# p768lwy3/torecsys

Measured on AMD Instinct MI355X. Metric: CTR samples/sec fwd+bwd (DeepFM, 39 fields x dim 64), higher is better.
Workload: dtype bf16; 1 GPU; BASELINE.json configs[1]: DeepFM 39 Criteo-shaped fields, MLP [400,400,400], 1000000 total rows, embed_dim 64, batch 65536, uniform indices, uniform field sizes; global_batch=65536, rows=1000000, parallelism=single, microbatches=1, optimizer=none, hipgraph=True, hipgraph_input_sets=1, hipgraph_steps_per_replay=4, fused_lookup_fm=True

## Files before the change

include/trs_abi.h:

```cpp
#ifndef TRS_ABI_H_
#define TRS_ABI_H_

#include <stddef.h>
#include <stdint.h>

#ifdef __cplusplus
extern "C" {
#endif

#define TRS_ABI_VERSION 3

enum { TRS_F32 = 0, TRS_BF16 = 1 };
enum { TRS_I64 = 0, TRS_I32 = 1 };
enum {
  TRS_OK = 0,
  TRS_EINVAL = -1,
  TRS_EDTYPE = -2,
  TRS_ESHAPE = -3,
  TRS_EALIGN = -4,
  TRS_ELAUNCH = -5,
  TRS_EWORKSPACE = -6
};

typedef void* trs_stream_t;
// ... 154 lines not shown
int trs_mlp_fused_fwd(const void* x, int64_t rows, int32_t num_layers, const int32_t* widths,
                      const void* const* weights, const void* const* biases, void* const* hidden, void* const* masks,
                      void* mask_in, void* y, int32_t dtype, int32_t family, int32_t x_stride, void* workspace,
                      size_t ws_bytes, trs_stream_t stream);
int trs_mlp_fused_bwd_data(const void* gy, int64_t rows, int32_t num_layers, const int32_t* widths,
                           const void* const* weights, const void* const* masks, void* const* gz, float* const* gbias,
                           void* gx, const void* mask_in, float* gbias_in, int32_t dtype, int32_t family,
                           void* workspace, size_t ws_bytes, trs_stream_t stream);

int trs_pad_cols(const void* src, int32_t c_in, void* dst, int32_t c_out, int64_t rows, int32_t dtype,
                 trs_stream_t stream);

size_t trs_rows_gemm_workspace_bytes(int32_t out_f, int32_t in_f);
int trs_rows_gemm_supported(int32_t out_f, int32_t in_f, int32_t x_stride);
int trs_rows_gemm(const void* x, int64_t rows, int32_t x_stride, const void* W, int32_t out_f, int32_t in_f,
                  int32_t dtype, void* y, void* workspace, size_t ws_bytes, trs_stream_t stream);

size_t trs_bucket_workspace_bytes(int64_t BN, int32_t world);
int trs_bucket_by_owner(const void* idx, int32_t idx_dtype, const int64_t* offsets, int64_t B, int32_t N,
                        int64_t rows_per_rank, int32_t world, int64_t* counts, int32_t* send_ids,
                        int32_t* send_pos, int32_t* inv_pos, void* workspace, size_t ws_bytes,
                        trs_stream_t stream);
int trs_embed_fm_sharded(const void* back, int64_t back_rows, const void* local, int64_t local_rows, int64_t n_valid,
                         int32_t E, int32_t dtype, const int32_t* inv_pos, const int32_t* send_ids, int32_t self_lo,
                         int32_t self_n, int64_t B, int32_t N, void* emb, void* fm, float* fm_sum, int32_t* err_flag,
                         trs_stream_t stream);
int trs_permute_grad(const void* g_block, const void* g_fm, const float* fm_sum, const void* x,
                     const int32_t* pos, int64_t K, int32_t N, int32_t E, int32_t dtype, void* out,
                     trs_stream_t stream);

int trs_rowdot_fwd(const void* h, const void* w, const void* bias, int64_t rows, int32_t C, int32_t dtype, void* out,
                   trs_stream_t stream);
size_t trs_rowdot_bwd_workspace_bytes(int64_t rows, int32_t C);
int trs_rowdot_bwd(const void* g, const void* h, const void* w, int64_t rows, int32_t C, int32_t dtype, void* gh,
                   float* gw, float* gb, void* workspace, size_t ws_bytes, trs_stream_t stream);

int trs_transpose_pad(const void* in, int64_t B, int32_t R, int32_t Cc, int32_t ld_in, void* out, int32_t ld_out,
                      int32_t dtype, trs_stream_t stream);

int trs_cat_head_fwd(const void* a, const void* d, const void* w, const void* bias, int64_t rows, int32_t N, int32_t Ea,
                     int32_t Eb, int32_t dtype, void* out, trs_stream_t stream);
size_t trs_cat_head_bwd_workspace_bytes(int64_t rows, int32_t N, int32_t Ea, int32_t Eb);
int trs_cat_head_bwd(const void* g, const void* a, const void* d, const void* w, int64_t rows, int32_t N, int32_t Ea,
                     int32_t Eb, int32_t dtype, void* ga, void* gd, float* gw, float* gb, void* workspace,
                     size_t ws_bytes, trs_stream_t stream);

int trs_wgrad_finish(const float* part, int32_t S, int32_t R, int32_t Cc, int32_t out_rows, int32_t out_cols,
                     int32_t dtype, void* gw, const float* gb_f32, void* gb, trs_stream_t stream);
int trs_wgrad_finish_t(const float* part, int32_t S, int32_t Cc, int32_t R, int32_t out_rows, int32_t out_cols,
                       int32_t dtype, void* gw, const float* gb_f32, void* gb, trs_stream_t stream);
int32_t trs_wgrad_rows_splits(int32_t M, int32_t N, int64_t rows);
int trs_wgrad_rows(const void* g, int32_t ldg, const void* x, int32_t ldx, int64_t rows, int32_t M, int32_t N,
                   int32_t dtype, int32_t S, float* part, trs_stream_t stream);
int trs_copy_padded_many(const int64_t* desc, int32_t n, int32_t elem_size, int64_t max_elems, trs_stream_t stream);

int32_t trs_cin_glue_blocks(int64_t B);
int trs_cin_glue_stats(const void* y, int64_t B, int32_t E, int32_t C, int32_t dtype, float* partial,
                       trs_stream_t stream);
int trs_cin_glue_fwd(const void* y, const float* scale, const float* shift, int64_t B, int32_t E, int32_t C, int32_t D,
                     int32_t Hs, int32_t dtype, void* hidden, void* pooled, trs_stream_t stream);
int trs_cin_glue_bwd_reduce(const void* y, const void* g_hidden, const void* g_pooled, const float* scale,
                            const float* shift, const float* mean, const float* invstd, int64_t B, int32_t E, int32_t C,
                            int32_t D, int32_t Hs, int32_t dtype, float* partial, trs_stream_t stream);
int trs_cin_glue_bwd_apply(const void* y, const void* g_hidden, const void* g_pooled, const float* scale,
                           const float* shift, const float* mean, const float* invstd, const float* c1, const float* c2,
                           int64_t B, int32_t E, int32_t C, int32_t D, int32_t Hs, int32_t dtype, void* gy,
                           trs_stream_t stream);
int trs_cin_glue_cf_supported(int32_t E, int32_t C);
int trs_cin_glue_fwd_cf(const void* y, const float* scale, const float* shift, int64_t B, int32_t E, int32_t C,
                        int32_t D, int32_t Hs, int32_t dtype, void* hidden, void* hidden_cf, void* pooled,
                        trs_stream_t stream);
int trs_cin_glue_bwd_apply_cf(const void* y, const void* g_hidden, const void* g_pooled, const float* scale,
                              const float* shift, const float* mean, const float* invstd, const float* c1,
                              const float* c2, int64_t B, int32_t E, int32_t C, int32_t D, int32_t Hs, int32_t dtype,
                              void* gy, void* gy_cf, float* colsum_partial, trs_stream_t stream);

int trs_opn_vec_fwd(const void* x, const void* kern, int32_t kern_is_num, int64_t B, int32_t N, int32_t E,
                    int32_t dtype, void* out, trs_stream_t stream);
size_t trs_opn_vec_bwd_workspace_bytes(int64_t B, int32_t N, int32_t E);
int trs_opn_vec_bwd(const void* g, const void* x, const void* kern, int32_t kern_is_num, int64_t B, int32_t N,
                    int32_t E, int32_t dtype, void* gx, float* gkern_vec, void* workspace, size_t ws_bytes,
                    trs_stream_t stream);

int trs_pair_mul_fwd(const void* a, const void* c, const void* bias, int32_t bias_per_pair, int64_t B, int32_t N,
                     int32_t E, int32_t dtype, void* out, trs_stream_t stream);
int trs_pair_mul_bwd(const void* g, const void* a, const void* c, int64_t B, int32_t N, int32_t E, int32_t dtype,
                     void* ga, void* gc, trs_stream_t stream);

int trs_rows_mul_bias_fwd(const void* a, const void* c, const void* bias, int32_t bias_per_pair, int64_t rows,
                          int32_t P, int32_t E, int32_t dtype, void* out, trs_stream_t stream);
int trs_rows_mul_bwd(const void* g, const void* a, const void* c, int64_t rows, int32_t E, int32_t dtype, void* ga,
                     void* gc, trs_stream_t stream);

int trs_pair_bilinear_fwd(const void* x, const void* W, int32_t w_per_pair, const void* bias, int32_t bias_per_pair,
                          int32_t mode, int64_t B, int32_t N, int32_t E, int32_t dtype, void* out,
                          trs_stream_t stream);
int trs_pair_bilinear_bwd_data(const void* g, const void* x, const void* W, int32_t w_per_pair, int32_t mode,
                               int64_t B, int32_t N, int32_t E, int32_t dtype, void* gx, void* gT,
                               trs_stream_t stream);

int trs_pair_bilinear_fwd_mfma(const void* x, const void* Wt, const void* bias, const int32_t* tasks, int32_t ntasks,
                               int32_t mode, int64_t B, int32_t N, int32_t E, int32_t dtype, void* out,
                               trs_stream_t stream);

int trs_pair_bilinear_bwd_data_mfma(const void* g, const void* x, const void* W, const void* Wt,
                                    const int32_t* tasks_i, int32_t nti, const int32_t* seg_i,
// ... 78 lines not shown
```

torecsys_amd/_abi.py:

```python
from __future__ import annotations

import ctypes
import os
import threading
from ctypes import c_char_p, c_int32, c_int64, c_size_t, c_void_p

import torch

_HERE = os.path.dirname(os.path.abspath(__file__))
LIB_PATH = os.environ.get("TRS_LIB_PATH") or os.path.join(_HERE, "libtrs_hip.so")

TRS_F32, TRS_BF16 = 0, 1
TRS_I64, TRS_I32 = 0, 1

_P, _I32, _I64, _SZ, _F32 = c_void_p, c_int32, c_int64, c_size_t, ctypes.c_float

_OPTIMIZER_TAIL = [_I32, _F32, _P, _F32, _F32, _F32, _P, _P, _P, _SZ, _P]

SIGNATURES = {
    "trs_version": (c_int32, []),
    "trs_last_error_string": (c_char_p, []),
    "trs_rowdot_fwd": (c_int32, [_P, _P, _P, _I64, _I32, _I32, _P, _P]),
    "trs_rowdot_bwd_workspace_bytes": (_SZ, [_I64, _I32]),
    "trs_rowdot_bwd": (c_int32, [_P, _P, _P, _I64, _I32, _I32, _P, _P, _P, _P, _SZ, _P]),
    "trs_transpose_pad": (c_int32, [_P, _I64, _I32, _I32, _I32, _P, _I32, _I32, _P]),
    "trs_cat_head_fwd": (c_int32, [_P, _P, _P, _P, _I64, _I32, _I32, _I32, _I32, _P, _P]),
    "trs_cat_head_bwd_workspace_bytes": (_SZ, [_I64, _I32, _I32, _I32]),
    "trs_cat_head_bwd": (c_int32, [_P, _P, _P, _P, _I64, _I32, _I32, _I32, _I32, _P, _P, _P, _P, _P, _SZ, _P]),
    "trs_wgrad_finish": (c_int32, [_P, _I32, _I32, _I32, _I32, _I32, _I32, _P, _P, _P, _P]),
    "trs_wgrad_finish_t": (c_int32, [_P, _I32, _I32, _I32, _I32, _I32, _I32, _P, _P, _P, _P]),
    "trs_wgrad_rows_splits": (c_int32, [_I32, _I32, _I64]),
    "trs_wgrad_rows": (c_int32, [_P, _I32, _P, _I32, _I64, _I32, _I32, _I32, _I32, _P, _P]),
    "trs_copy_padded_many": (c_int32, [_P, _I32, _I32, _I64, _P]),
    "trs_cin_glue_blocks": (c_int32, [_I64]),
    "trs_cin_glue_stats": (c_int32, [_P, _I64, _I32, _I32, _I32, _P, _P]),
    "trs_cin_glue_fwd": (c_int32, [_P, _P, _P, _I64, _I32, _I32, _I32, _I32, _I32, _P, _P, _P]),
    "trs_cin_glue_bwd_reduce": (c_int32, [_P, _P, _P, _P, _P, _P, _P, _I64, _I32, _I32, _I32, _I32, _I32, _P, _P]),
    "trs_cin_glue_bwd_apply": (c_int32, [_P, _P, _P, _P, _P, _P, _P, _P, _P, _I64, _I32, _I32, _I32, _I32, _I32, _P, _P]),
    "trs_cin_glue_cf_supported": (c_int32, [_I32, _I32]),
    "trs_cin_glue_fwd_cf": (c_int32, [_P, _P, _P, _I64, _I32, _I32, _I32, _I32, _I32, _P, _P, _P, _P]),
    "trs_cin_glue_bwd_apply_cf": (c_int32, [_P, _P, _P, _P, _P, _P, _P, _P, _P, _I64, _I32, _I32, _I32, _I32, _I32, _P, _P, _P,
                                            _P]),
    "trs_opn_vec_fwd": (c_int32, [_P, _P, _I32, _I64, _I32, _I32, _I32, _P, _P]),
    "trs_opn_vec_bwd_workspace_bytes": (_SZ, [_I64, _I32, _I32]),
    "trs_opn_vec_bwd": (c_int32, [_P, _P, _P, _I32, _I64, _I32, _I32, _I32, _P, _P, _P, _SZ, _P]),
    "trs_pair_mul_fwd": (c_int32, [_P, _P, _P, _I32, _I64, _I32, _I32, _I32, _P, _P]),
    "trs_rows_mul_bias_fwd": (c_int32, [_P, _P, _P, _I32, _I64, _I32, _I32, _I32, _P, _P]),
    "trs_rows_mul_bwd": (c_int32, [_P, _P, _P, _I64, _I32, _I32, _P, _P, _P]),
    "trs_pair_mul_bwd": (c_int32, [_P, _P, _P, _I64, _I32, _I32, _I32, _P, _P, _P]),
    "trs_pair_bilinear_fwd": (c_int32, [_P, _P, _I32, _P, _I32, _I32, _I64, _I32, _I32, _I32, _P, _P]),
    "trs_pair_bilinear_bwd_data": (c_int32, [_P, _P, _P, _I32, _I32, _I64, _I32, _I32, _I32, _P, _P, _P]),
    "trs_pair_bilinear_fwd_mfma": (c_int32, [_P, _P, _P, _P, _I32, _I32, _I64, _I32, _I32, _I32, _P, _P]),
    "trs_pair_bilinear_bwd_data_mfma": (c_int32, [_P, _P, _P, _P, _P, _I32, _P, _P, _I32, _P, _I32, _I64, _I32, _I32, _I32,
                                                  _P, _P, _P, _P]),
    "trs_pair_bilinear_bwd_w_mfma_workspace_bytes": (_SZ, [_I64, _I32, _I32]),
    "trs_pair_bilinear_bwd_w_mfma": (c_int32, [_P, _P, _I32, _I64, _I32, _I32, _I32, _P, _P, _SZ, _P]),
    "trs_pair_epilogue_fwd": (c_int32, [_P, _P, _P, _I32, _I32, _I64, _I32, _I32, _I32, _P, _P]),
    "trs_pair_epilogue_bwd": (c_int32, [_P, _P, _P, _I32, _I64, _I32, _I32, _I32, _P, _P]),
    "trs_afm_fwd_dropout": (c_int32, [_P, _P, _P, _P, _P, _P, _F32, _I64, _I32, _I32, _I32, _I32, _P, _P, _P, _P]),
    "trs_afm_bwd_dropout": (c_int32, [_P, _P, _P, _P, _P, _F32, _P, _P, _P, _I64, _I32, _I32, _I32, _I32, _P, _P, _P, _P,
                                      _P, _P, _SZ, _P]),
    "trs_afm_pair_tiles": (c_int32, [_I32, _P, _I32, _P]),
    "trs_pad_cols": (c_int32, [_P, _I32, _P, _I32, _I64, _I32, _P]),
    "trs_rows_gemm_workspace_bytes": (_SZ, [_I32, _I32]),
    "trs_rows_gemm_supported": (c_int32, [_I32, _I32, _I32]),
    "trs_rows_gemm": (c_int32, [_P, _I64, _I32, _P, _I32, _I32, _I32, _P, _P, _SZ, _P]),
    "trs_afm_bwd_workspace_bytes": (_SZ, [_I64, _I32, _I32, _I32]),
    "trs_pack_columns": (c_int32, [_P, _P, _I32, _I32, _I64, _P, _I32, _P]),
    "trs_mark_timestamp": (c_int32, [_P, _I32, _P]),
    "trs_wall_clock_khz": (_I64, []),
    "trs_gather_rows": (c_int32, [_P, _I64, _I32, _I32, _P, _I32, _P, _I64, _I32, _P, _P, _P]),
    "trs_gather_rows_tables": (c_int32, [_P, _P, _I32, _I32, _P, _I32, _I64, _I32, _P, _P, _P]),
    "trs_fa_gather_rows": (c_int32, [_P, _I64, _I32, _I32, _P, _I32, _P, _I64, _I32, _P, _P, _P]),
    "trs_csr_workspace_bytes": (_SZ, [_I64, _I64]),
    "trs_csr_build": (c_int32, [_P, _I32, _P, _I64, _I32, _I64, _P, _P, _P, _SZ, _P, _P]),
    "trs_csr_build_skip": (c_int32, [_P, _I32, _P, _I64, _I32, _I64, _I64, _P, _P, _P, _SZ, _P, _P]),
    "trs_scatter_workspace_bytes": (_SZ, [_I64, _I32, _I32, _I32]),
    "trs_scatter_rows": (c_int32, [_P, _I64, _P, _I32, _P, _P, _P, _P, _I64, _I64, _I32, _I32, _I32, _I64, _P, _P, _SZ, _P]),
    "trs_scatter_rows_first": (c_int32, [_P, _I64, _P, _I32, _P, _P, _P, _P, _I64, _I64, _I32, _I32, _I32, _I64, _P, _P, _P, _P,
                                         _SZ, _P]),
    "trs_scatter_rows_update": (c_int32, [_P, _I64, _P, _I32, _P, _P, _P, _P, _I64, _I64, _I32, _I32, _I32, _I64,
                                          *_OPTIMIZER_TAIL]),
    "trs_scatter_rows_update_mapped": (c_int32, [_P, _P, _P, _P, _P, _I64, _I64, _I64, _I32, _I32, *_OPTIMIZER_TAIL]),
    "trs_adam_step_size": (c_int32, [_P, _P, ctypes.c_double, ctypes.c_double, _P, _P]),
    "trs_compact_rows_slots": (_I64, [_I64]),
# ... 281 lines not shown
```

torecsys_amd/csrc/wgrad_rows.hip:

```cpp
#include <algorithm>

#include "trs_common.hpp"

namespace trs {

typedef __attribute__((ext_vector_type(4))) short wg_s16x4;
typedef __attribute__((ext_vector_type(8))) short wg_s16x8;
typedef __attribute__((ext_vector_type(8))) __bf16 wg_bf16x8;
typedef __attribute__((ext_vector_type(4))) float wg_f32x4;

constexpr int WG_KR = 64;
constexpr int WG_KS = 32;
constexpr int WG_PANEL = WG_KS * 32 + 32;
constexpr int WG_TC = 7;

struct WgradArgs {
  const uint16_t* g;
  const uint16_t* x;
  float* part;
  int64_t rows;
  int ldg, ldx;
  int M, N;
  int MB, NB;
  int slots_per_xcd;
};

__host__ __device__ __forceinline__ int split_start(int total, int parts, int k) { return (int)(((int64_t)total * k) / parts); }

__device__ __forceinline__ wg_bf16x8 tr_frag(const char* lo_p, const char* hi_p, int off) {
  typedef __attribute__((address_space(3))) wg_s16x4* lds_p;
  const wg_s16x4 lo = __builtin_amdgcn_ds_read_tr16_b64_v4i16((lds_p)(lo_p + off));
  const wg_s16x4 hi = __builtin_amdgcn_ds_read_tr16_b64_v4i16((lds_p)(hi_p + off));
  const wg_s16x8 v = {lo[0], lo[1], lo[2], lo[3], hi[0], hi[1], hi[2], hi[3]};
  return __builtin_bit_cast(wg_bf16x8, v);
}

__device__ __forceinline__ void wg_mfma(wg_f32x4& acc, const wg_bf16x8& A, const wg_bf16x8& B) {
  asm volatile("v_mfma_f32_16x16x32_bf16 %0, %1, %2, %0" : "+a"(acc) : "v"(A), "v"(B));
}

template <int WM, int WN, int MC, int NC, bool CHECK>
__global__ __launch_bounds__(64 * WM * WN, 1) void wgrad_rows_kernel(WgradArgs a) {
  constexpr int NWAVES = WM * WN;
  constexpr bool EXACT = NWAVES == 8;
  extern __shared__ __attribute__((aligned(16))) char wg_lds[];
  const int lane = threadIdx.x & 63, wave = __builtin_amdgcn_readfirstlane(threadIdx.x >> 6);
  const int q = lane >> 4, i = lane & 15;
  const bool odd = q & 1;

  const int TB = a.MB * a.NB;
  const int xcd = blockIdx.x & 7, j = blockIdx.x >> 3;
  const int slot = xcd * a.slots_per_xcd + j / TB;
  const int S = 8 * a.slots_per_xcd;
  const int tile = j % TB;
  const int mb = tile / a.NB, nb = tile % a.NB;
  const int Mt = (a.M + 15) >> 4, Nt = (a.N + 15) >> 4;
  const int bm0 = split_start(Mt, a.MB, mb), bm1 = split_start(Mt, a.MB, mb + 1);
  const int bn0 = split_start(Nt, a.NB, nb), bn1 = split_start(Nt, a.NB, nb + 1);
  const int PM = bm1 - bm0, PN = bn1 - bn0, P = PM + PN;
  const int wm = wave / WN, wn = (EXACT && wave >= 4) ? ((wave + 1) & 3) : wave % WN;
  const int am0 = split_start(PM, WM, wm), mc = split_start(PM, WM, wm + 1) - am0;
  const int an0 = split_start(PN, WN, wn), nc = split_start(PN, WN, wn + 1) - an0;
  const int64_t quads_total = (a.rows + 4 * WG_KS - 1) / (4 * WG_KS);
  const int64_t h0 = 4 * (quads_total * slot / S), h1 = 4 * (quads_total * (slot + 1) / S);
  const int64_t n_h = h1 - h0;

  constexpr int NLD = 32 / NWAVES;
  const int panel = (wave & 3) * 8 + ((lane & 15) >> 1);
  const int rlow = (wave >> 2) * 16 + (lane >> 4), half = lane & 1;
  const bool is_g = panel < PM;
  const int col = is_g ? 16 * (bm0 + panel) + 8 * half : 16 * (bn0 + panel - PM) + 8 * half;
  const bool col_ok = panel < P && col + 8 <= (is_g ? a.M : a.N);
  const int ld = is_g ? a.ldg : a.ldx;
  const uint16_t* src = (is_g ? a.g : a.x) + col;
  const int lds_off = panel * WG_PANEL + rlow * 32 + half * 16;
  const int slot_bytes = P * WG_PANEL;

// ... 219 lines not shown
      }                                                                                                             \
      landed();                                                                                                     \
      cur = nx;                                                                                                     \
    }
    if (n_h > 0) {
#pragma unroll
      for (int k = 0; k < WD_AHEAD; ++k) issue(k, k);
      landed();
      {
        const char* cb = wg_lds;
#pragma unroll
        for (int n = 0; n < NCx; ++n) Bf[n] = tr_frag(cb + b_lo, cb + b_hi, n * 32);
#pragma unroll
        for (int m = 0; m < PD; ++m) Ar[m] = tr_frag(cb + a_lo, cb + a_hi, m * 32);
      }
      for (int64_t k = 0; k < n_h; k += 4) {
        WD_STEP(0, k)
        WD_STEP(1, k + 1)
        WD_STEP(2, k + 2)
        WD_STEP(3, k + 3)
      }
    }
#undef WD_STEP
    asm volatile("s_waitcnt vmcnt(0)\n\ts_nop 15\n\ts_nop 15" ::: "memory");
    float* out = a.part + (int64_t)slot * a.M * a.N;
#pragma unroll
    for (int m = 0; m < MCx; ++m)
#pragma unroll
      for (int n = 0; n < NCx; ++n)
        if (m < mc && n < nc) {
          const int row = 16 * (bm0 + am0 + m) + 4 * q, c = 16 * (bn0 + an0 + n) + i;
#pragma unroll
          for (int e = 0; e < 4; ++e)
            if (row + e < a.M && c < a.N) out[(int64_t)(row + e) * a.N + c] = acc[m][n][e];
        }
  };
  if (mc == MC && nc == NC) run.template operator()<MC, NC>();
  else if (mc == MC) run.template operator()<MC, NC - 1>();
  else if (nc == NC) run.template operator()<MC - 1, NC>();
  else run.template operator()<MC - 1, NC - 1>();
}

constexpr int WD2_SLOT = 3 * WD_IMG;
constexpr int WD2_NSLOT = 4;
constexpr int WD2_AHEAD = 3;
constexpr int64_t WD2_MIN_ROWS = 1 << 20;

template <bool AG>
__device__ __forceinline__ void wd_mfma(wg_f32x4& acc, const wg_bf16x8& A, const wg_bf16x8& B) {
  if constexpr (AG) asm volatile("v_mfma_f32_16x16x32_bf16 %0, %1, %2, %0" : "+a"(acc) : "v"(A), "v"(B));
  else asm volatile("v_mfma_f32_16x16x32_bf16 %0, %1, %2, %0" : "+v"(acc) : "v"(A), "v"(B));
}

__global__ __launch_bounds__(256, 1) void wgrad_dma2_kernel(WgradArgs a) {
  extern __shared__ __attribute__((aligned(16))) char wg_lds[];
  const int lane = threadIdx.x & 63, wave = __builtin_amdgcn_readfirstlane(threadIdx.x >> 6);
  const int q = lane >> 4, i = lane & 15;
  const bool odd = q & 1;
  const int TB = a.MB;
  const int xcd = blockIdx.x & 7, j = blockIdx.x >> 3;
  const int slot = xcd * a.slots_per_xcd + j / TB;
  const int S = 8 * a.slots_per_xcd;
  const int mb = j % TB;
  const int Mt = (a.M + 15) >> 4, Nt = (a.N + 15) >> 4;
  const int bm0 = split_start(Mt, a.MB, mb), PM = split_start(Mt, a.MB, mb + 1) - bm0;
  const int xb = wave >> 1;
  const int bn0 = split_start(Nt, 2, xb), PN = split_start(Nt, 2, xb + 1) - bn0;
  const int an0 = split_start(PN, 2, wave & 1), nc = split_start(PN, 2, (wave & 1) + 1) - an0;
  const int xc0 = 16 * split_start(Nt, 2, 0), xc1 = 16 * split_start(Nt, 2, 1);
  const int64_t quads_total = a.rows / (4 * WG_KS);
  const int64_t h0 = 4 * (quads_total * slot / S), h1 = 4 * (quads_total * (slot + 1) / S);
  const int64_t n_h = h1 - h0;

  const char* gcol = reinterpret_cast<const char*>(a.g + 16 * bm0);
  const char* x0col = reinterpret_cast<const char*>(a.x + xc0);
  const char* x1col = reinterpret_cast<const char*>(a.x + xc1);
  unsigned voff[10];
#pragma unroll
  for (int t = 0; t < 10; ++t) {
    const int p = wave + 4 * t, img = p / 13, jj = p - 13 * img;
    const int o = jj * 1024 + 16 * lane, row = o / WD_S, cb = o - row * WD_S;
    voff[t] = (unsigned)(row * (img ? a.ldx : a.ldg) * 2 + cb);
  }
  const unsigned lds0 = (unsigned)(uintptr_t)(__attribute__((address_space(3))) const char*)wg_lds;
  auto issue = [&](int64_t k, unsigned ring_slot) __attribute__((always_inline)) {
    const int64_t h = h0 + (k < n_h ? k : n_h - 1);
    const char* gs = gcol + h * WG_KS * a.ldg * 2;
    const char* x0s = x0col + h * WG_KS * a.ldx * 2;
    const char* x1s = x1col + h * WG_KS * a.ldx * 2;
    const unsigned base = lds0 + ring_slot * WD2_SLOT;
#pragma unroll
    for (int t = 0; t < 10; ++t) {
      const int p = wave + 4 * t;
      if (p < 39) wd_dma(p < 13 ? gs : (p < 26 ? x0s : x1s), voff[t], base + p * 1024);
    }
  };
  auto landed = [&]() __attribute__((always_inline)) {
    if (wave < 3) asm volatile("s_waitcnt vmcnt(10) lgkmcnt(0)\n\ts_barrier" ::: "memory");
    else asm volatile("s_waitcnt vmcnt(9) lgkmcnt(0)\n\ts_barrier" ::: "memory");
  };

  auto run = [&]<int MCx, int NCx>() __attribute__((always_inline)) {
    wg_f32x4 acc[MCx][NCx];
#pragma unroll
    for (int m = 0; m < MCx; ++m)
#pragma unroll
      for (int n = 0; n < NCx; ++n) acc[m][n] = wg_f32x4{0.f, 0.f, 0.f, 0.f};
    const int frag_lane = (8 * q + (i >> 2)) * WD_S + (i & 3) * 8;
    const int a_lo = frag_lane + (odd ? 4 * WD_S : 0), a_hi = frag_lane + (odd ? 0 : 4 * WD_S);
    const int b_lo = WD_IMG * (1 + xb) + an0 * 32 + frag_lane + (odd ? 4 * WD_S : 0);
    const int b_hi = WD_IMG * (1 + xb) + an0 * 32 + frag_lane + (odd ? 0 : 4 * WD_S);
    constexpr int PD = 2;
    wg_bf16x8 Ar[4], Bf[NCx];
#define WD2_STEP(c4, KEXPR)                                                                                         \
    {                                                                                                               \
      const char* cb = wg_lds + (c4) * WD2_SLOT;                                                                    \
// ... 70 lines not shown
    if (p.MB * p.NB > 32) return WgradPlan{0, 0, 0, 0, 0, 0, 0};
    if (((Nt + p.NB - 1) / p.NB + 1) / 2 <= 5) p.nc = 5;
    const int pm_lo = Mt / p.MB, pm_hi = (Mt + p.MB - 1) / p.MB, pn_lo = Nt / p.NB, pn_hi = (Nt + p.NB - 1) / p.NB;
    if (pm_lo >= 12 && pm_hi <= 14 && pn_lo >= 12 && pn_hi <= 16) {
      p.wn = 4;
      p.mc = 7;
      p.nc = 4;
    } else if (pm_lo >= 12 && pm_hi <= 14 && pn_lo >= 8 && pn_hi <= 12) {
      p.wn = 4;
      p.mc = 7;
      p.nc = 3;
    }
  }
  auto blocks_ok = [](int T, int B, int cols) {
    for (int b = 0; b < B; ++b) {
      const int t0 = split_start(T, B, b), t1 = split_start(T, B, b + 1);
      if (t1 - t0 < 12 || t1 - t0 > 13 || 16 * t0 + 208 > cols) return false;
    }
    return true;
  };
  if (p.wm == 2 && p.wn == 4 && p.nc == 4 && rows % (4 * WG_KS) == 0 && blocks_ok(Mt, p.MB, M) &&
      blocks_ok(Nt, p.NB, N))
    p.dma = (p.NB == 2 && rows >= WD2_MIN_ROWS) ? 2 : 1;
  int slots = 32 / (p.dma == 2 ? p.MB : p.MB * p.NB);
  const int64_t stages = (rows + WG_KR - 1) / WG_KR;
  while (slots > 1 && stages / (8 * slots) < 4) slots >>= 1;
  p.slots_per_xcd = slots;
  return p;
}

template <int WM, int WN, int MC, int NC, bool CHECK>
int wgrad_launch_c(const WgradArgs& a, int grid, size_t lds, hipStream_t s) {
  static bool attr = false;
  if (!attr) {
    if (hipFuncSetAttribute((const void*)wgrad_rows_kernel<WM, WN, MC, NC, CHECK>, hipFuncAttributeMaxDynamicSharedMemorySize,
                            160 * 1024) != hipSuccess)
      return check_launch("wgrad_rows: LDS attribute");
    attr = true;
  }
  hipLaunchKernelGGL((wgrad_rows_kernel<WM, WN, MC, NC, CHECK>), dim3(grid), dim3(64 * WM * WN), lds, s, a);
  return check_launch("wgrad_rows");
}

}

using namespace trs;

template <int WM, int WN, int MC, int NC>
static int wgrad_launch(const WgradArgs& a, int grid, size_t lds, hipStream_t s) {
  return (a.rows % (4 * WG_KS)) ? wgrad_launch_c<WM, WN, MC, NC, true>(a, grid, lds, s)
                          : wgrad_launch_c<WM, WN, MC, NC, false>(a, grid, lds, s);
}

extern "C" int32_t trs_wgrad_rows_splits(int32_t M, int32_t N, int64_t rows) {
  const WgradPlan p = wgrad_plan(M, N, rows);
  return 8 * p.slots_per_xcd;
}

extern "C" int trs_wgrad_rows(const void* g, int32_t ldg, const void* x, int32_t ldx, int64_t rows, int32_t M, int32_t N,
                              int32_t dtype, int32_t S, float* part, trs_stream_t stream) {
  TRS_REQUIRE(dtype == TRS_BF16, TRS_EDTYPE, "wgrad_rows: bf16 operands only");
  WgradPlan p = wgrad_plan(M, N, rows);
  TRS_REQUIRE(p.slots_per_xcd > 0 && S == 8 * p.slots_per_xcd, TRS_ESHAPE,
              "wgrad_rows: (M=%d, N=%d, rows=%lld) takes %d row ranges, caller passed %d", M, N, (long long)rows,
              8 * p.slots_per_xcd, S);
  TRS_REQUIRE(ldg >= M && ldx >= N && (ldg & 7) == 0 && (ldx & 7) == 0 && aligned16(g) && aligned16(x), TRS_ESHAPE,
              "wgrad_rows: row strides must be multiples of 8 elements and cover M / N, operands 16-byte aligned");
  if (!g || !x || !part) return fail(TRS_EINVAL, "wgrad_rows: null pointer");
  hipStream_t s = (hipStream_t)stream;
  WgradArgs a{(const uint16_t*)g, (const uint16_t*)x, part, rows, ldg, ldx, M, N, p.MB, p.NB, p.slots_per_xcd};
  const int Mt = (M + 15) / 16, Nt = (N + 15) / 16;
  const int PM = (Mt + p.MB - 1) / p.MB, PN = (Nt + p.NB - 1) / p.NB;
  const size_t lds = (size_t)(4 * (PM + PN) + WG_TC) * WG_PANEL;
  const int grid = 8 * p.slots_per_xcd * p.MB * p.NB;
  TRS_REQUIRE(p.dma == 0 || (int64_t)WG_KS * std::max(ldg, ldx) * 2 < ((int64_t)1 << 31), TRS_ESHAPE, "wgrad_rows: row stride too large");
  if (p.dma == 2) {
    static bool attr2 = false;
    if (!attr2) {
      if (hipFuncSetAttribute((const void*)wgrad_dma2_kernel, hipFuncAttributeMaxDynamicSharedMemorySize, 160 * 1024) != hipSuccess)
        return check_launch("wgrad_rows(dma2): LDS attribute");
      attr2 = true;
    }
    hipLaunchKernelGGL(wgrad_dma2_kernel, dim3(8 * p.slots_per_xcd * p.MB), dim3(256), (size_t)WD2_NSLOT * WD2_SLOT, s, a);
    return check_launch("wgrad_rows(dma2)");
  }
  if (p.dma == 1) {
    static bool attr = false;
    if (!attr) {
      if (hipFuncSetAttribute((const void*)wgrad_dma_kernel<7, 4>, hipFuncAttributeMaxDynamicSharedMemorySize, 160 * 1024) != hipSuccess)
        return check_launch("wgrad_rows(dma): LDS attribute");
      attr = true;
    }
    hipLaunchKernelGGL((wgrad_dma_kernel<7, 4>), dim3(grid), dim3(512), (size_t)WD_NSLOT * WD_SLOT, s, a);
    return check_launch("wgrad_rows(dma)");
  }
  if (p.wm == 2 && p.wn == 4)
    return p.nc == 4 ? wgrad_launch<2, 4, 7, 4>(a, grid, lds, s) : wgrad_launch<2, 4, 7, 3>(a, grid, lds, s);
  if (p.wm == 2)
    return p.nc == 5 ? wgrad_launch<2, 2, WG_TC, 5>(a, grid, lds, s) : wgrad_launch<2, 2, WG_TC, WG_TC>(a, grid, lds, s);
  if (p.wm == 4) return p.nc == 4 ? wgrad_launch<4, 1, WG_TC, 4>(a, grid, lds, s) : wgrad_launch<4, 1, WG_TC, WG_TC>(a, grid, lds, s);
  if (p.mc == 1) return wgrad_launch<1, 4, 1, WG_TC>(a, grid, lds, s);
  if (p.mc == 4) return wgrad_launch<1, 4, 4, WG_TC>(a, grid, lds, s);
  return wgrad_launch<1, 4, WG_TC, WG_TC>(a, grid, lds, s);
}
```

torecsys_amd/layers.py:

```python
from __future__ import annotations

from abc import ABC, abstractmethod
from typing import Dict, List, Optional, Tuple

import math
import os

import torch
import torch.nn as nn

from . import functional as F_


def _strip(t: torch.Tensor) -> torch.Tensor:
    return t.rename(None) if t.has_names() else t


class BaseLayer(nn.Module, ABC):

    def __init__(self, **kwargs):
        super().__init__()

    @property
    @abstractmethod
# ... 583 lines not shown
    def forward(ctx, x, weight, bias, fuse_relu, w_pad, b_pad):
        W = weight if w_pad is None else w_pad
        Bv = bias if w_pad is None else b_pad
        x2 = x.reshape(-1, x.shape[-1])
        if fuse_relu and Bv is not None and x2.is_cuda:
            y = torch._addmm_activation(Bv, x2, W.t(), use_gelu=False).reshape(*x.shape[:-1], W.shape[0])
        else:
            y = torch.nn.functional.linear(x, W, Bv)
            if fuse_relu:
                y = torch.relu_(y)
        ctx.has_bias = bias is not None
        ctx.fuse_relu = bool(fuse_relu) and bias is not None and F_.relu_bwd_bias_supported(y.reshape(-1, y.shape[-1]))
        ctx.relu = bool(fuse_relu)
        ctx.wshape = tuple(weight.shape)
        ctx.wdtype = weight.dtype
        ctx.save_for_backward(x, W, y if fuse_relu else None)
        return y

    @staticmethod
    def backward(ctx, g):
        x, W, y = ctx.saved_tensors
        out_f, in_f = ctx.wshape
        gx = gw = gb = None
        if ctx.fuse_relu:
            gz, gbf = F_.relu_bwd_bias(g.reshape(-1, g.shape[-1]), y.reshape(-1, y.shape[-1]))
            g = gz.reshape(g.shape)
            gb = gbf[:out_f].to(ctx.wdtype)
        elif ctx.relu:
            g = g * (y > 0).to(g.dtype)
        g2 = g.reshape(-1, g.shape[-1])
        x2 = x.reshape(-1, x.shape[-1])
        if ctx.needs_input_grad[0]:
            gx = (g2 @ W).reshape(x.shape)
        if ctx.needs_input_grad[1]:
            rows, S = g2.shape[0], _split_count(g2.shape[0], _LinearSplitK.SPLIT_ROWS)
            if S >= 4 and rows % S == 0 and 32 <= g2.shape[1] <= 1024 and 32 <= x2.shape[1] <= 1024 \
                    and g2.is_contiguous() and x2.is_contiguous():
                part = torch.bmm(g2.view(S, rows // S, -1).transpose(1, 2), x2.view(S, rows // S, -1),
                                 out_dtype=torch.float32)
                gw = part.sum(0)[:out_f, :in_f].to(ctx.wdtype)
            else:
                gw = (g2.t() @ x2)[:out_f, :in_f]
                if not gw.is_contiguous():
                    gw = gw.contiguous()
        if ctx.has_bias and ctx.needs_input_grad[2] and gb is None:
            rows = g2.shape[0]
            if g2.shape[1] <= 8 and rows % 1024 == 0 and rows >= 8192 and g2.is_contiguous():
                gb = g2.view(rows // 1024, 1024, -1).float().sum(1).sum(0)[:out_f].to(g2.dtype)
            else:
                gb = g2.sum(0)[:out_f]
        return gx, gw, gb, None, None, None


def _dense_layer_grads(g2, gbf, xin, W, out_f, in_f, wdt, need_x, need_w, need_b):
    rows = xin.shape[0]
    gw_out = gb_out = None
    S = _split_count(rows, _LinearSplitK.SPLIT_ROWS)
    if need_w or (need_b and gbf is not None):
        if need_w and S >= 4 and rows % S == 0 and 32 <= g2.shape[1] <= 1024 and 32 <= xin.shape[1] <= 4096 \
                and xin.is_contiguous():
            gw = torch.empty(out_f, in_f, dtype=wdt, device=xin.device)
            St = _split_count(rows, _MLPStack.SPLIT_ROWS_WIDE)
            if xin.shape[1] >= 2 * g2.shape[1] and St >= 4:
                part = torch.bmm(xin.view(St, rows // St, -1).transpose(1, 2), g2.view(St, rows // St, -1),
                                 out_dtype=torch.float32)
                with_b = need_b and gbf is not None
                gb = torch.empty(out_f, dtype=wdt, device=xin.device) if with_b else None
                F_.call("trs_wgrad_finish_t", F_.ptr(part), St, part.shape[1], part.shape[2], out_f, in_f,
                        F_.value_dtype_code(gw), F_.ptr(gw), F_.ptr(gbf) if with_b else F_.ptr(None), F_.ptr(gb),
                        F_.stream_ptr())
            else:
                part = torch.bmm(g2.view(S, rows // S, -1).transpose(1, 2), xin.view(S, rows // S, -1),
                                 out_dtype=torch.float32)
                with_b = need_b and gbf is not None and out_f <= (in_f + 255) // 256 * 256
                gb = torch.empty(out_f, dtype=wdt, device=xin.device) if with_b else None
                F_.call("trs_wgrad_finish", F_.ptr(part), S, part.shape[1], part.shape[2], out_f, in_f,
                        F_.value_dtype_code(gw), F_.ptr(gw), F_.ptr(gbf) if with_b else F_.ptr(None), F_.ptr(gb),
                        F_.stream_ptr())
            gw_out = gw
            if with_b:
                gb_out = gb
        elif need_w:
            gw = (g2.t() @ xin)[:out_f, :in_f]
            gw_out = gw if gw.is_contiguous() else gw.contiguous()
    if need_b and gb_out is None:
        gb_out = gbf[:out_f].to(wdt) if gbf is not None else g2.sum(0)[:out_f]
    gx = None
    if need_x and F_.rows_gemm_supported(g2, W, out_f, xin.shape[1]) and W.shape[1] == xin.shape[1]:
        gx = F_.rows_gemm(g2, W, out_f, xin.shape[1])
    elif need_x:
        gx = g2 @ W
    return gx, gw_out, gb_out


class _HybridMLP(torch.autograd.Function):

    @staticmethod
    def forward(ctx, x, w_narrow, *tensors):
        cur = x.reshape(-1, x.shape[-1])
        w1, b1, w1u, b1u = tensors[:4]
        tail = tensors[4:]
        W1 = w1 if w1u is None else w1u
        B1 = b1 if w1u is None else b1u
        L = len(tail) // 4
        Ws = [(tail[4 * l] if tail[4 * l + 2] is None else tail[4 * l + 2]).contiguous() for l in range(L)]
        bs = [(tail[4 * l + 1] if tail[4 * l + 3] is None else tail[4 * l + 3]).contiguous() for l in range(L)]
        h1 = torch._addmm_activation(B1, cur, W1.t(), use_gelu=False)
        if w_narrow is not None:
            y, hidden, masks, mask_in, fam = F_.fused_mlp_forward_raw(h1, [w_narrow] + Ws[1:], bs, input_mask=True,
                                                                      family=F_.MLP_FAMILY_MIXED, x_stride=h1.shape[1])
        else:
            y, hidden, masks, mask_in, fam = F_.fused_mlp_forward_raw(h1, Ws, bs, input_mask=True)
# ... 425 lines not shown
```

Before: 58.94 million samples/s.

## Route wide first-layer MLP weight gradient through custom dma2 split-K kernel

```diff
diff --git a/include/trs_abi.h b/include/trs_abi.h
--- a/include/trs_abi.h
+++ b/include/trs_abi.h
@@ -230,6 +230,9 @@
 int32_t trs_wgrad_rows_splits(int32_t M, int32_t N, int64_t rows);
 int trs_wgrad_rows(const void* g, int32_t ldg, const void* x, int32_t ldx, int64_t rows, int32_t M, int32_t N,
                    int32_t dtype, int32_t S, float* part, trs_stream_t stream);
+int32_t trs_wgrad_wide_splits(int32_t M_x, int32_t N_g, int32_t ld_g, int64_t rows);
+int trs_wgrad_wide(const void* x, int32_t ldx, const void* g, int32_t ldg, int64_t rows, int32_t M_x, int32_t N_g,
+                   int32_t S, float* part, trs_stream_t stream);
 int trs_copy_padded_many(const int64_t* desc, int32_t n, int32_t elem_size, int64_t max_elems, trs_stream_t stream);
 
 int32_t trs_cin_glue_blocks(int64_t B);
diff --git a/torecsys_amd/_abi.py b/torecsys_amd/_abi.py
--- a/torecsys_amd/_abi.py
+++ b/torecsys_amd/_abi.py
@@ -31,6 +31,8 @@
     "trs_wgrad_finish_t": (c_int32, [_P, _I32, _I32, _I32, _I32, _I32, _I32, _P, _P, _P, _P]),
     "trs_wgrad_rows_splits": (c_int32, [_I32, _I32, _I64]),
     "trs_wgrad_rows": (c_int32, [_P, _I32, _P, _I32, _I64, _I32, _I32, _I32, _I32, _P, _P]),
+    "trs_wgrad_wide_splits": (c_int32, [_I32, _I32, _I32, _I64]),
+    "trs_wgrad_wide": (c_int32, [_P, _I32, _P, _I32, _I64, _I32, _I32, _I32, _P, _P]),
     "trs_copy_padded_many": (c_int32, [_P, _I32, _I32, _I64, _P]),
     "trs_cin_glue_blocks": (c_int32, [_I64]),
     "trs_cin_glue_stats": (c_int32, [_P, _I64, _I32, _I32, _I32, _P, _P]),
diff --git a/torecsys_amd/csrc/wgrad_rows.hip b/torecsys_amd/csrc/wgrad_rows.hip
--- a/torecsys_amd/csrc/wgrad_rows.hip
+++ b/torecsys_amd/csrc/wgrad_rows.hip
@@ -23,6 +23,7 @@
   int M, N;
   int MB, NB;
   int slots_per_xcd;
+  int S;
 };
 
 __host__ __device__ __forceinline__ int split_start(int total, int parts, int k) { return (int)(((int64_t)total * k) / parts); }
@@ -348,16 +349,27 @@
   else asm volatile("v_mfma_f32_16x16x32_bf16 %0, %1, %2, %0" : "+v"(acc) : "v"(A), "v"(B));
 }
 
+__device__ __forceinline__ void wd2_place(const WgradArgs& a, int b, int& slot, int& mb) {
+  const int xcd = b & 7, j = b >> 3, local = a.slots_per_xcd * a.MB;
+  if (j < local) {
+    slot = xcd * a.slots_per_xcd + j / a.MB;
+    mb = j % a.MB;
+  } else {
+    const int r = (j - local) * 8 + xcd;
+    slot = 8 * a.slots_per_xcd + r / a.MB;
+    mb = r % a.MB;
+  }
+}
+
 __global__ __launch_bounds__(256, 1) void wgrad_dma2_kernel(WgradArgs a) {
   extern __shared__ __attribute__((aligned(16))) char wg_lds[];
   const int lane = threadIdx.x & 63, wave = __builtin_amdgcn_readfirstlane(threadIdx.x >> 6);
   const int q = lane >> 4, i = lane & 15;
   const bool odd = q & 1;
-  const int TB = a.MB;
-  const int xcd = blockIdx.x & 7, j = blockIdx.x >> 3;
-  const int slot = xcd * a.slots_per_xcd + j / TB;
-  const int S = 8 * a.slots_per_xcd;
-  const int mb = j % TB;
+  const int S = a.S;
+  int slot, mb;
+  wd2_place(a, blockIdx.x, slot, mb);
+  if (slot >= S) return;
   const int Mt = (a.M + 15) >> 4, Nt = (a.N + 15) >> 4;
   const int bm0 = split_start(Mt, a.MB, mb), PM = split_start(Mt, a.MB, mb + 1) - bm0;
   const int xb = wave >> 1;
@@ -534,6 +546,17 @@
                           : wgrad_launch_c<WM, WN, MC, NC, false>(a, grid, lds, s);
 }
 
+static int wgrad_dma2_launch(const WgradArgs& a, int grid, hipStream_t s, const char* what) {
+  static bool attr2 = false;
+  if (!attr2) {
+    if (hipFuncSetAttribute((const void*)wgrad_dma2_kernel, hipFuncAttributeMaxDynamicSharedMemorySize, 160 * 1024) != hipSuccess)
+      return check_launch("wgrad_dma2: LDS attribute");
+    attr2 = true;
+  }
+  hipLaunchKernelGGL(wgrad_dma2_kernel, dim3(grid), dim3(256), (size_t)WD2_NSLOT * WD2_SLOT, s, a);
+  return check_launch(what);
+}
+
 extern "C" int32_t trs_wgrad_rows_splits(int32_t M, int32_t N, int64_t rows) {
   const WgradPlan p = wgrad_plan(M, N, rows);
   return 8 * p.slots_per_xcd;
@@ -550,21 +573,15 @@
               "wgrad_rows: row strides must be multiples of 8 elements and cover M / N, operands 16-byte aligned");
   if (!g || !x || !part) return fail(TRS_EINVAL, "wgrad_rows: null pointer");
   hipStream_t s = (hipStream_t)stream;
-  WgradArgs a{(const uint16_t*)g, (const uint16_t*)x, part, rows, ldg, ldx, M, N, p.MB, p.NB, p.slots_per_xcd};
+  WgradArgs a{(const uint16_t*)g, (const uint16_t*)x, part, rows, ldg, ldx, M, N, p.MB, p.NB, p.slots_per_xcd, 0};
   const int Mt = (M + 15) / 16, Nt = (N + 15) / 16;
   const int PM = (Mt + p.MB - 1) / p.MB, PN = (Nt + p.NB - 1) / p.NB;
   const size_t lds = (size_t)(4 * (PM + PN) + WG_TC) * WG_PANEL;
   const int grid = 8 * p.slots_per_xcd * p.MB * p.NB;
   TRS_REQUIRE(p.dma == 0 || (int64_t)WG_KS * std::max(ldg, ldx) * 2 < ((int64_t)1 << 31), TRS_ESHAPE, "wgrad_rows: row stride too large");
   if (p.dma == 2) {
-    static bool attr2 = false;
-    if (!attr2) {
-      if (hipFuncSetAttribute((const void*)wgrad_dma2_kernel, hipFuncAttributeMaxDynamicSharedMemorySize, 160 * 1024) != hipSuccess)
-        return check_launch("wgrad_rows(dma2): LDS attribute");
-      attr2 = true;
-    }
-    hipLaunchKernelGGL(wgrad_dma2_kernel, dim3(8 * p.slots_per_xcd * p.MB), dim3(256), (size_t)WD2_NSLOT * WD2_SLOT, s, a);
-    return check_launch("wgrad_rows(dma2)");
+    a.S = 8 * p.slots_per_xcd;
+    return wgrad_dma2_launch(a, a.S * p.MB, s, "wgrad_rows(dma2)");
   }
   if (p.dma == 1) {
     static bool attr = false;
@@ -585,3 +602,38 @@
   if (p.mc == 4) return wgrad_launch<1, 4, 4, WG_TC>(a, grid, lds, s);
   return wgrad_launch<1, 4, WG_TC, WG_TC>(a, grid, lds, s);
 }
+
+struct WidePlan {
+  int spx, S, grid;
+};
+
+static WidePlan wide_plan(int MB) {
+  WidePlan w{std::min(32 / MB, 4), 0, 0};
+  const int extra = w.spx == 32 / MB ? 8 * (32 - w.spx * MB) / MB : 0;
+  w.S = 8 * w.spx + extra;
+  w.grid = 8 * (w.spx * MB + (extra * MB + 7) / 8);
+  return w;
+}
+
+extern "C" int32_t trs_wgrad_wide_splits(int32_t M_x, int32_t N_g, int32_t ld_g, int64_t rows) {
+  if (M_x < 2 * 208 || M_x % 208 || N_g < 8 || (N_g & 15) || (ld_g & 7) || rows <= 0 || rows % (4 * WG_KS)) return 0;
+  const int Nt = N_g / 16, MB = M_x / 208;
+  if (Nt < 24 || Nt > 26 || 16 * split_start(Nt, 2, 1) + 208 > ld_g || MB > 32) return 0;
+  if ((int64_t)WG_KS * std::max(M_x, ld_g) * 2 >= ((int64_t)1 << 31)) return 0;
+  const int S = wide_plan(MB).S;
+  return rows >= (int64_t)4 * WG_KS * S ? S : 0;
+}
+
+extern "C" int trs_wgrad_wide(const void* x, int32_t ldx, const void* g, int32_t ldg, int64_t rows, int32_t M_x, int32_t N_g,
+                              int32_t S, float* part, trs_stream_t stream) {
+  if (!g || !x || !part) return fail(TRS_EINVAL, "wgrad_wide: null pointer");
+  TRS_REQUIRE(ldx >= M_x && (ldx & 7) == 0 && aligned16(g) && aligned16(x) && (int64_t)WG_KS * ldx * 2 < ((int64_t)1 << 31),
+              TRS_ESHAPE, "wgrad_wide: operands 16-byte aligned, ldx a multiple of 8 elements that covers M_x, under 2^31 bytes per 32 rows");
+  const int S0 = trs_wgrad_wide_splits(M_x, N_g, ldg, rows);
+  TRS_REQUIRE(S0 > 0 && S == S0, TRS_ESHAPE, "wgrad_wide: (M_x=%d, N_g=%d, ldg=%d, rows=%lld) takes %d row ranges, caller passed %d",
+              M_x, N_g, ldg, (long long)rows, S0, S);
+  const int MB = M_x / 208;
+  const WidePlan w = wide_plan(MB);
+  WgradArgs a{(const uint16_t*)x, (const uint16_t*)g, part, rows, ldx, ldg, M_x, N_g, MB, 2, w.spx, S};
+  return wgrad_dma2_launch(a, w.grid, (hipStream_t)stream, "wgrad_wide");
+}
diff --git a/torecsys_amd/layers.py b/torecsys_amd/layers.py
--- a/torecsys_amd/layers.py
+++ b/torecsys_amd/layers.py
@@ -659,12 +659,37 @@
         return gx, gw, gb, None, None, None
 
 
+WIDE_WGRAD_MIN_ROWS = 6144
+
+
+def _wide_wgrad_splits(g2, xin, out_f, in_f) -> int:
+    if not (xin.shape[0] >= WIDE_WGRAD_MIN_ROWS and g2.dtype == xin.dtype == torch.bfloat16
+            and xin.shape[1] == in_f and g2.shape[1] >= out_f
+            and g2.stride(1) == 1 and xin.stride(1) == 1 and xin.stride(0) % 8 == 0
+            and g2.data_ptr() % 16 == 0 and xin.data_ptr() % 16 == 0):
+        return 0
+    return F_.size_query("trs_wgrad_wide_splits", in_f, out_f, g2.stride(0), xin.shape[0])
+
+
 def _dense_layer_grads(g2, gbf, xin, W, out_f, in_f, wdt, need_x, need_w, need_b):
     rows = xin.shape[0]
     gw_out = gb_out = None
     S = _split_count(rows, _LinearSplitK.SPLIT_ROWS)
     if need_w or (need_b and gbf is not None):
-        if need_w and S >= 4 and rows % S == 0 and 32 <= g2.shape[1] <= 1024 and 32 <= xin.shape[1] <= 4096 \
+        Sw = _wide_wgrad_splits(g2, xin, out_f, in_f) if need_w else 0
+        if Sw:
+            gw = torch.empty(out_f, in_f, dtype=wdt, device=xin.device)
+            part = torch.empty(Sw, in_f, out_f, dtype=torch.float32, device=xin.device)
+            F_.call("trs_wgrad_wide", F_.ptr(xin), xin.stride(0), F_.ptr(g2), g2.stride(0), rows, in_f, out_f, Sw,
+                    F_.ptr(part), F_.stream_ptr())
+            with_b = need_b and gbf is not None
+            gb = torch.empty(out_f, dtype=wdt, device=xin.device) if with_b else None
+            F_.call("trs_wgrad_finish_t", F_.ptr(part), Sw, in_f, out_f, out_f, in_f, F_.value_dtype_code(gw),
+                    F_.ptr(gw), F_.ptr(gbf) if with_b else F_.ptr(None), F_.ptr(gb), F_.stream_ptr())
+            gw_out = gw
+            if with_b:
+                gb_out = gb
+        elif need_w and S >= 4 and rows % S == 0 and 32 <= g2.shape[1] <= 1024 and 32 <= xin.shape[1] <= 4096 \
                 and xin.is_contiguous():
             gw = torch.empty(out_f, in_f, dtype=wdt, device=xin.device)
             St = _split_count(rows, _MLPStack.SPLIT_ROWS_WIDE)
```

Measured after the change: 60.84 million samples/s (median of 6 runs). +3.2%, better.
